# abowman6/CBET_RayTracing_3D

Hardware: AMD Instinct MI355X
Metric: ray-steps/sec, OMEGA 60-beam 256^3 sweep (higher is better)
Workload: dtype f64

## Files before the change

### cbet_raytracing_3d_amd/api.py

```python
import ctypes as C
import os

import numpy as np

_PKG = os.path.dirname(os.path.abspath(__file__))
LIB_PATH = os.environ.get("CBET_LIB_PATH") or os.path.join(_PKG, "lib", "libcbet_mi355x.so")
DATA_DIR = os.path.join(_PKG, "data")

OK, EINVAL, EHIP, ENOMEM, ENODEVICE, ECOMM = 0, -1, -2, -3, -4, -5
NPHASE = 2001
KERNEL_DEFAULT, KERNEL_GLOBAL_ATOMICS, KERNEL_LDS_COMBINE, KERNEL_LDS_WINDOW = 0, 1, 2, 3


class CbetError(RuntimeError):
    def __init__(self, code, msg):
        super().__init__("cbet error %d: %s" % (code, msg))
        self.code = code


class Params(C.Structure):
    _fields_ = [
        ("nx", C.c_int), ("ny", C.c_int), ("nz", C.c_int),
        ("xmin", C.c_double), ("xmax", C.c_double),
        ("ymin", C.c_double), ("ymax", C.c_double),
# ... 94 lines not shown

    def idx(c, n):
        c = np.where(c > 0.0, c, 0.0)
        return np.minimum(np.floor(c), n - 1).astype(np.int64)

    hist = np.zeros((ntheta, nphi))
    np.add.at(hist, (idx(ct, ntheta), idx(cp, nphi)), r["uray"])
    return hist


EXPORTS = [
    "cbet_last_error", "cbet_version", "cbet_params_default", "cbet_derive",
    "cbet_live_ray_list", "cbet_omega60_beam_norm", "cbet_host_power_table", "cbet_host_beam_trig", "cbet_read_profile",
    "cbet_safeGPUAlloc", "cbet_moveToAndFromGPU", "cbet_gpuFree",
    "cbet_context_create", "cbet_context_destroy", "cbet_context_counters", "cbet_context_tables", "cbet_context_set_launch_list",
    "cbet_launch_ray_XYZ", "cbet_tabulate_plasma", "cbet_trace_nodes", "cbet_prepare_step_records", "cbet_ray_tracing",
    "cbet_write_text", "cbet_edep_average", "cbet_edep_average_device", "cbet_node_coordinates", "cbet_write_npy",
    "cbet_debug_bounds_violations",
    "cbet_gain_params_default", "cbet_gain_constants", "cbet_trace_cbet", "cbet_gain_field",
    "cbet_cbet_workspace_bytes", "cbet_cbet_solve", "cbet_gain_field_slab", "cbet_gain_field_packed",
    "cbet_cbet_slab_workspace_bytes", "cbet_cbet_slab_workspace_bytes_parts", "cbet_pack_segments", "cbet_unpack_segments",
    "cbet_context_list_length", "cbet_cbet_workspace_gain", "cbet_trace_exits", "cbet_exit_tally", "cbet_farfield",
    "cbet_sph_modes_device", "cbet_sph_modes", "cbet_prepare_plasma", "cbet_context_step_records",
]

_lib = None


def lib():
    global _lib
    if _lib is not None:
        return _lib
    import torch
    if not os.path.exists(LIB_PATH):
        raise ImportError(
            "%s is missing: build it with `python -m cbet_raytracing_3d_amd.build` "
            "(hipcc --offload-arch=gfx950).  There is no CPU fallback." % LIB_PATH)
    L = C.CDLL(LIB_PATH)
    vp, dp, ip = C.c_void_p, C.POINTER(C.c_double), C.POINTER(C.c_int)
    L.cbet_last_error.restype = C.c_char_p
    L.cbet_version.restype = C.c_char_p
    L.cbet_params_default.argtypes = [C.POINTER(Params), C.c_int]
    L.cbet_derive.argtypes = [C.POINTER(Params), C.POINTER(Derived)]
    L.cbet_live_ray_list.argtypes = [C.POINTER(Params), ip, C.c_long, C.POINTER(C.c_long)]
    L.cbet_omega60_beam_norm.restype = dp
    L.cbet_host_power_table.argtypes = [dp, dp]
    L.cbet_host_beam_trig.argtypes = [dp, C.c_int, dp]
    L.cbet_read_profile.argtypes = [C.c_char_p, C.c_int, dp, dp]
    L.cbet_safeGPUAlloc.argtypes = [C.POINTER(vp), C.c_size_t, C.c_int]
    L.cbet_moveToAndFromGPU.argtypes = [vp, vp, C.c_size_t, C.c_int]
    L.cbet_gpuFree.argtypes = [vp, C.c_int]
    L.cbet_context_create.argtypes = [C.POINTER(vp), C.POINTER(Params), C.c_int]
    L.cbet_context_destroy.argtypes = [vp]
    L.cbet_context_counters.argtypes = [vp, vp, C.POINTER(Counters), C.c_int]
    L.cbet_context_set_launch_list.argtypes = [vp, ip, C.c_long]
    L.cbet_context_tables.argtypes = [vp, C.POINTER(vp), C.POINTER(vp)]
    L.cbet_launch_ray_XYZ.argtypes = [C.c_int, C.c_uint, vp, vp, vp, vp, vp, vp, vp, vp,
                                      C.c_double, C.c_double, C.c_double, C.POINTER(Params), vp, vp]
    L.cbet_tabulate_plasma.argtypes = [vp, C.POINTER(Params), vp, vp, vp, vp]
    L.cbet_prepare_step_records.argtypes = [vp, C.POINTER(Params), vp, vp, C.c_double, C.c_double, C.c_double, vp]
    L.cbet_prepare_plasma.argtypes = [vp, C.POINTER(Params), vp, vp, vp, C.c_double, C.c_double, C.c_double, vp]
    L.cbet_context_step_records.argtypes = [vp, C.POINTER(vp), C.POINTER(C.c_ulonglong)]
    L.cbet_trace_nodes.argtypes = [C.c_int, C.c_uint, vp, vp, vp, vp, vp, vp, vp,
                                   C.c_double, C.c_double, C.c_double, C.POINTER(Params), vp, vp]
    L.cbet_ray_tracing.argtypes = [dp, dp, dp, dp, C.POINTER(Params), dp, ip, C.c_int, dp,
                                   C.POINTER(Counters)]
    L.cbet_debug_bounds_violations.argtypes = [C.POINTER(C.c_ulonglong), C.c_int, vp]
    L.cbet_write_text.argtypes = [dp, C.c_int, C.c_int, C.c_int, C.c_char_p]
    L.cbet_write_text.restype = C.c_longlong
    L.cbet_edep_average.argtypes = [dp, dp, C.c_int, C.c_int, C.c_int]
    L.cbet_edep_average_device.argtypes = [vp, vp, C.c_int, C.c_int, C.c_int, vp]
    L.cbet_node_coordinates.argtypes = [C.POINTER(Params), dp, dp, dp]
    L.cbet_write_npy.argtypes = [dp, C.c_int, C.POINTER(C.c_long), C.c_char_p]
    L.cbet_write_npy.restype = C.c_longlong
    L.cbet_gain_params_default.argtypes = [C.POINTER(GainParams)]
    L.cbet_gain_constants.argtypes = [C.POINTER(Params), C.POINTER(GainParams), dp, dp, dp]
    L.cbet_trace_cbet.argtypes = [C.c_int, C.c_uint, vp, vp, vp, C.c_int, vp, vp, vp, vp, vp, vp,
                                  C.c_double, C.c_double, C.c_double, C.POINTER(Params), C.POINTER(GainParams), vp, vp]
    L.cbet_gain_field.argtypes = [vp, vp, vp, vp, vp, C.POINTER(Params), C.POINTER(GainParams), vp, vp]
    L.cbet_gain_field_slab.argtypes = [vp, vp, vp, vp, vp, C.c_int, C.c_int, C.POINTER(Params), C.POINTER(GainParams), vp, vp]
    L.cbet_gain_field_packed.argtypes = [vp, vp, vp, vp, vp, C.c_int, C.c_int, C.POINTER(Params), C.POINTER(GainParams), vp, vp]
    L.cbet_pack_segments.argtypes = [vp, C.c_long, C.c_int, C.c_int, vp, C.c_long, vp, vp]
    L.cbet_unpack_segments.argtypes = [vp, C.c_long, C.c_int, C.c_int, vp, C.c_long, vp, vp]
    L.cbet_cbet_slab_workspace_bytes.argtypes = [C.POINTER(Params), C.c_int, C.c_int]
    L.cbet_cbet_slab_workspace_bytes.restype = C.c_size_t
# ... 145 lines not shown
        c = Counters()
        _check(lib().cbet_context_counters(self._h, _addr(stream), C.byref(c), 1 if reset else 0))
        return c

    def set_launch_list(self, slots):
        arr = np.ascontiguousarray(slots, dtype=np.int32)
        _check(lib().cbet_context_set_launch_list(self._h, arr.ctypes.data_as(C.POINTER(C.c_int)), arr.size))

    def list_length(self):
        n = C.c_long()
        _check(lib().cbet_context_list_length(self._h, C.byref(n)))
        return n.value

    def tables(self):
        a, b = C.c_void_p(), C.c_void_p()
        _check(lib().cbet_context_tables(self._h, C.byref(a), C.byref(b)))
        return a.value, b.value

    def step_records(self):
        a, n = C.c_void_p(), C.c_ulonglong()
        _check(lib().cbet_context_step_records(self._h, C.byref(a), C.byref(n)))
        return a.value, n.value

    def close(self):
        if self._h:
            lib().cbet_context_destroy(self._h)
            self._h = C.c_void_p()

    def __del__(self):
        try:
            self.close()
        except Exception:
            pass


def launch_ray_XYZ(b, nindices, te_data_g, r_data_g, ne_data_g, edep, bbeam_norm, beam_norm, pow_r,
                   phase_r, xconst, yconst, zconst, params, ctx=None, stream=None):
    _check(lib().cbet_launch_ray_XYZ(
        b, nindices, _addr(te_data_g), _addr(r_data_g), _addr(ne_data_g), _addr(edep),
        _addr(bbeam_norm), _addr(beam_norm), _addr(pow_r), _addr(phase_r), xconst, yconst, zconst,
        C.byref(params), ctx.handle if ctx is not None else None, _addr(stream)))


def tabulate_plasma(ctx, params, te_data_g, r_data_g, ne_data_g, stream=None):
    _check(lib().cbet_tabulate_plasma(ctx.handle, C.byref(params), _addr(te_data_g),
                                      _addr(r_data_g), _addr(ne_data_g), _addr(stream)))
# ... 207 lines not shown
```

### cbet_raytracing_3d_amd/build.py

```python
import os
import shutil
import subprocess
import sys

PKG = os.path.dirname(os.path.abspath(__file__))
ROOT = os.path.dirname(PKG)
CSRC = os.path.join(PKG, "csrc")
LIB_DIR = os.path.join(PKG, "lib")
LIB_PATH = os.path.join(LIB_DIR, "libcbet_mi355x.so")
SOURCES = ["cbet_kernels.hip", "cbet_trace_window.hip", "cbet_trace_exit.hip", "cbet_grid_kernels.hip", "cbet_sph_modes.hip",
           "cbet_abi.cpp", "cbet_host.cpp", "cbet_output.cpp", "cbet_sph_host.cpp"]
HEADERS = [os.path.join(CSRC, "cbet_device.h"), os.path.join(CSRC, "cbet_relocate.h"), os.path.join(CSRC, "cbet_trace_common.h"), os.path.join(ROOT, "include", "cbet_mi355x.h"),
           os.path.join(ROOT, "include", "cbet_omega_beams.h")]

FLAGS = ["-O3", "-std=c++17", "--offload-arch=gfx950", "-ffp-contract=off", "-fPIC", "-shared",
         "-Wall", "-Wextra", "-Wno-unused-result", "-mllvm", "-structurizecfg-skip-uniform-regions=true"]


def hipcc():
    exe = shutil.which("hipcc") or "/opt/rocm/bin/hipcc"
    if not os.path.exists(exe):
        raise RuntimeError("hipcc not found (need ROCm to build the gfx950 library)")
    return exe


def is_stale():
    if not os.path.exists(LIB_PATH):
        return True
    built = os.path.getmtime(LIB_PATH)
    deps = [os.path.join(CSRC, s) for s in SOURCES] + HEADERS + [os.path.abspath(__file__),
                                                                os.path.join(ROOT, "tools", "cbet_gpu.cpp"),
                                                                os.path.join(ROOT, "tools", "cbet_reference_shaped.cpp"),
                                                                os.path.join(ROOT, "include", "cbet_reference_api.hpp")]
    return any(os.path.getmtime(d) > built for d in deps)

# ... 67 lines not shown
```

### cbet_raytracing_3d_amd/csrc/cbet_abi.cpp

```cpp
#include <hip/hip_runtime_api.h>

#include <algorithm>
#include <cmath>
#include <cstdarg>
#include <cstdio>
#include <cstdlib>
#include <cstring>
#include <map>
#include <mutex>
#include <vector>

#include "cbet_device.h"
#include "cbet_mi355x.h"
#include "cbet_omega_beams.h"

namespace cbet {

thread_local char g_err[512] = "";

int fail(int code, const char *fmt, ...)
{
    va_list ap;
    va_start(ap, fmt);
    vsnprintf(g_err, sizeof g_err, fmt, ap);
    va_end(ap);
    if (code == CBET_EHIP || code == CBET_ENODEVICE || code == CBET_ENOMEM) (void)hipGetLastError();
    return code;
}

#define CBET_HIP(call)                                                                          \
    do {                                                                                        \
        hipError_t e_ = (call);                                                                 \
        if (e_ != hipSuccess)                                                                   \
            return ::cbet::fail(CBET_EHIP, "%s failed: %s", #call, hipGetErrorString(e_));      \
    } while (0)
// ... 191 lines not shown
    xl = launch_axis(d->nrays_x, d->nrays_x, d->dx / 2);
    yl = launch_axis(d->nrays_y, d->nrays_y, d->dy / 2);
    long ntraced = 0, nlive = 0;
    build_live_list(p, d, d->nindices, xl, yl, live, ntraced, nlive);
    d->ntraced_ids = ntraced;
    d->nlive_rays = nlive;
    return CBET_OK;
}

}

using namespace cbet;

struct cbet_context {
    int gpu = -1;
    cbet_params p{};
    cbet_derived d{};
    double *ne3d = nullptr, *kap3d = nullptr;
    StepRecord *steprec = nullptr;
    unsigned long long tables_version = 0, rec_version = ~0ull;
    unsigned long long rec_builds = 0;
    const double *rec_ne3d = nullptr, *rec_kap3d = nullptr;
    double rec_const[3] = {0, 0, 0};
    double *xlaunch = nullptr, *ylaunch = nullptr;
    double *bounds = nullptr;
    int *live = nullptr;
    int nlive = 0;
    unsigned long long *counters = nullptr;
};

extern "C" {

const char *cbet_last_error(void) { return g_err; }
const char *cbet_version(void) { return "cbet-mi355x 0.1 (gfx950, hip)"; }

int cbet_params_default(cbet_params *p, int n)
{
    if (!p) return fail(CBET_EINVAL, "params is NULL");
    std::memset(p, 0, sizeof *p);
    p->nx = p->ny = p->nz = n;
    p->xmin = p->ymin = p->zmin = -0.13;
    p->xmax = p->ymax = p->zmax = 0.13;
    p->nbeams = 60;
    p->rays_per_zone = 4;
    p->courant_mult = 0.5;
    p->absorption = 1;
// ... 102 lines not shown
    if (e != hipSuccess) return fail(CBET_ENODEVICE, "hipSetDevice(%d): %s", gpu, hipGetErrorString(e));
    e = hipMemcpy(dst, src, size, hipMemcpyDefault);
    if (e != hipSuccess) return fail(CBET_EHIP, "Error encountered during hipMemcpy: %s", hipGetErrorString(e));
    return CBET_OK;
}

int cbet_gpuFree(void *ptr, int gpu)
{
    DeviceGuard guard;
    hipError_t e = hipSetDevice(gpu);
    if (e != hipSuccess) return fail(CBET_ENODEVICE, "hipSetDevice(%d): %s", gpu, hipGetErrorString(e));
    CBET_HIP(hipFree(ptr));
    return CBET_OK;
}

int cbet_context_destroy(cbet_context *ctx)
{
    if (!ctx) return CBET_OK;
    DeviceGuard guard;
    (void)hipSetDevice(ctx->gpu);
    (void)hipFree(ctx->ne3d);
    (void)hipFree(ctx->kap3d);
    (void)hipFree(ctx->steprec);
    (void)hipFree(ctx->xlaunch);
    (void)hipFree(ctx->ylaunch);
    (void)hipFree(ctx->bounds);
    (void)hipFree(ctx->live);
    (void)hipFree(ctx->counters);
    delete ctx;
    return CBET_OK;
}

int cbet_context_set_launch_list(cbet_context *ctx, const int *list, long n)
{
    if (!ctx || !list) return fail(CBET_EINVAL, "NULL context or list");
    if (n <= 0 || n % kWave != 0) return fail(CBET_EINVAL, "a launch list is a whole number of 64-entry bundles (got %ld entries)", n);
    DeviceGuard guard;
    CBET_HIP(hipSetDevice(ctx->gpu));
    CBET_HIP(hipDeviceSynchronize());
    std::vector<int> cur((size_t)ctx->nlive), want, got;
    if (ctx->nlive) CBET_HIP(hipMemcpy(cur.data(), ctx->live, cur.size() * sizeof(int), hipMemcpyDeviceToHost));
    for (int v : cur) if (v >= 0) want.push_back(v);
    for (long i = 0; i < n; ++i) {
        if (list[i] >= 0) got.push_back(list[i]);
        else if (list[i] != -1) return fail(CBET_EINVAL, "launch list entry %ld is %d (a ray id or -1)", i, list[i]);
    }
    for (long b = 0; b < n; b += kWave) {
        bool any = false;
        for (int l = 0; l < kWave; ++l) any = any || list[b + l] >= 0;
        if (!any) return fail(CBET_EINVAL, "bundle %ld of the launch list is empty", b / kWave);
    }
    std::sort(want.begin(), want.end());
    std::sort(got.begin(), got.end());
    if (want != got) return fail(CBET_EINVAL, "the launch list must hold exactly the context's live rays, each once (%zu given, %zu expected)", got.size(), want.size());
    int *fresh = nullptr;
    CBET_HIP(hipMalloc((void **)&fresh, (size_t)n * sizeof(int)));
    hipError_t e = hipMemcpy(fresh, list, (size_t)n * sizeof(int), hipMemcpyHostToDevice);
    if (e != hipSuccess) { (void)hipFree(fresh); return fail(CBET_EHIP, "hipMemcpy(launch list): %s", hipGetErrorString(e)); }
    (void)hipFree(ctx->live);
    ctx->live = fresh;
    ctx->nlive = (int)n;
    return CBET_OK;
}

int cbet_context_create(cbet_context **out, const cbet_params *p, int gpu)
{
    if (!out) return fail(CBET_EINVAL, "ctx out-pointer is NULL");
    *out = nullptr;
    if (int rc = validate(p)) return rc;
    cbet_derived d;
    std::vector<double> xl, yl;
    std::vector<int> live;
    if (int rc = derive_launch(p, &d, xl, yl, live)) return rc;

    DeviceGuard guard;
    hipError_t e = hipSetDevice(gpu);
    if (e != hipSuccess) return fail(CBET_ENODEVICE, "hipSetDevice(%d): %s", gpu, hipGetErrorString(e));
    cbet_context *ctx = new cbet_context;
    ctx->gpu = gpu;
    ctx->p = *p;
    ctx->d = d;
    ctx->nlive = (int)live.size();
    const size_t nodes = (size_t)p->nx * p->ny * p->nz;
    auto bail = [&](hipError_t err, const char *what) {
// ... 145 lines not shown
    if (int rc = check_geometry(ctx, p)) return rc;
    DeviceGuard guard;
    CBET_HIP(hipSetDevice(ctx->gpu));
    return step_records(ctx, p, ne3d, kappa3d, xconst, yconst, zconst, stream, true);
}

int cbet_prepare_plasma(cbet_context *ctx, const cbet_params *p, const double *te_data_g, const double *r_data_g,
                        const double *ne_data_g, double xconst, double yconst, double zconst, void *stream)
{
    if (!ctx) return fail(CBET_EINVAL, "NULL context");
    if (int rc = validate(p)) return rc;
    if (int rc = check_geometry(ctx, p)) return rc;
    if (!te_data_g || !r_data_g || !ne_data_g) return fail(CBET_EINVAL, "NULL profile pointer");
    if (plasma_records_lds(p->nprofile) > 65536) {
        if (int rc = cbet_tabulate_plasma(ctx, p, te_data_g, r_data_g, ne_data_g, stream)) return rc;
        return cbet_prepare_step_records(ctx, p, nullptr, nullptr, xconst, yconst, zconst, stream);
    }
    DeviceGuard guard;
    CBET_HIP(hipSetDevice(ctx->gpu));
    PlasmaRecordsArgs a{};
    a.t = tabulate_args(p, ctx, te_data_g, r_data_g, ne_data_g);
    a.xconst = xconst; a.yconst = yconst; a.zconst = zconst;
    a.rec = ctx->steprec;
    CBET_HIP(launch_plasma_records(a, (hipStream_t)stream));
    ++ctx->tables_version;
    ++ctx->rec_builds;
    ctx->rec_version = ctx->tables_version;
    ctx->rec_ne3d = ctx->ne3d; ctx->rec_kap3d = ctx->kap3d;
    ctx->rec_const[0] = xconst; ctx->rec_const[1] = yconst; ctx->rec_const[2] = zconst;
    return CBET_OK;
}

struct CbetHooks {
    const double *gain = nullptr;
    int quantity = 0;
    double *beam_gain = nullptr;
    double max_exponent = 0.0;
    bool exits = false;
};

static int trace_impl(int b, unsigned nindices, const double *ne3d, const double *kappa3d,
                      double *edep, const double *bbeam_norm, const double *beam_norm,
                      const double *pow_r, const double *phase_r, double xconst, double yconst,
                      double zconst, const cbet_params *p, cbet_context *ctx, void *stream,
                      const CbetHooks &hooks)
{
// ... 455 lines not shown
```

### cbet_raytracing_3d_amd/csrc/cbet_device.h

```cpp
#ifndef CBET_DEVICE_H_
#define CBET_DEVICE_H_

#include <hip/hip_runtime_api.h>

#include "cbet_mi355x.h"

namespace cbet {

constexpr double kC = 29979245800.0;
constexpr double kE0 = 8.85418782e-12;
constexpr double kMe = 9.10938356e-31;
constexpr double kEc = 1.60217662e-19;
constexpr double kLambda = 1.053e-4 / 3.0;
constexpr double kSigma = 0.0375;
constexpr double kIntensity = 1.0e14;
constexpr double kFocal = 0.1;
constexpr double kBeamMin = -450.0e-4;
constexpr double kBeamMax = 450.0e-4;

constexpr unsigned kEmptyTag = 0xFFFFFFFFu;
constexpr int kWave = 64;

enum CounterSlot { kCntSteps = 0, kCntRays = 1, kCntGlobalAtomics = 2, kCntEvictions = 3, kCntWaveSteps = 4,
                   kCntWaveStepsMiss = 5, kCntWaveStepsWide = 6, kCntSlabsRetired = 7, kCntSlots = 8 };
// ... 2 lines not shown
    int nx, ny, nz, nprofile;
    double xmin, ymin, zmin;
    double dx, dy, dz, dt;
    double ncrit;
    const double *r, *ne, *te;
    double *ne3d, *kap3d;
};

struct StepRecord {
    double kx, ky, kz, kap;
};

struct StepTableArgs {
    int nx, ny, nz;
    double xconst, yconst, zconst;
    const double *ne3d, *kap3d;
    StepRecord *rec;
};

struct PlasmaRecordsArgs {
    TabulateArgs t;
    double xconst, yconst, zconst;
    StepRecord *rec;
};

struct TraceArgs {
    int nx, ny, nz;
    double xmin, ymin, zmin;
    double dx, dy, dz, dt;
    double inv_dx, inv_dy, inv_dz;
    double fx_hi, fy_hi, fz_hi;
    const double *bounds;
    double tol_x, tol_y, tol_z;
    double xconst, yconst, zconst;
    int nt, absorption;
    int rpz, zones, nrays_x;
    double z_launch;
    double uray_mult, omega, ncrit;
    const double *xlaunch, *ylaunch;
    const int *live;
    int nlive;
    int beam_lo, nbeams_local, bundles_per_beam;
    long total_bundles;
    long first_item, item_count;
    const double *ne3d, *kap3d;
    const StepRecord *steprec;
// ... 73 lines not shown
```

### cbet_raytracing_3d_amd/csrc/cbet_kernels.hip

```cpp
#include <hip/hip_runtime.h>

#include "cbet_trace_common.h"

namespace cbet {
namespace {

__device__ __forceinline__ void interp_table2(const double *y1, const double *y2, const double *x, const double xp,
                                              int n, double &o1, double &o2)
{
    const bool ascending = x[0] <= x[n - 1];
    if (ascending ? (xp <= x[0]) : (xp >= x[0])) { o1 = y1[0]; o2 = y2[0]; return; }
    if (ascending ? (xp >= x[n - 1]) : (xp <= x[n - 1])) { o1 = y1[n - 1]; o2 = y2[n - 1]; return; }
    unsigned lo = 0, hi = n - 1, mid = (lo + hi) >> 1;
    while (lo < hi - 1) {
        const bool go_low = ascending ? (x[mid] >= xp) : !(x[mid] <= xp);
        if (go_low) hi = mid; else lo = mid;
        mid = (lo + hi) >> 1;
    }
    const double dx = x[mid + 1] - x[mid], t = xp - x[mid];
    o1 = y1[mid] + (y1[mid + 1] - y1[mid]) / dx * t;
    o2 = y2[mid] + (y2[mid + 1] - y2[mid]) / dx * t;
}

__device__ __forceinline__ void node_plasma(const TabulateArgs &a, const double *s_r, const double *s_ne, const double *s_te,
// ... 39 lines not shown
    const long sY = a.nz, sX = (long)a.ny * a.nz;
    for (long idx = (long)blockIdx.x * blockDim.x + threadIdx.x; idx < total; idx += stride) {
        const int k = (int)(idx % a.nz);
        const long ij = idx / a.nz;
        const int j = (int)(ij % a.ny);
        const int i = (int)(ij / a.ny);
        const long oxm = (i == 0) ? 0 : ((i == a.nx - 1) ? -2 * sX : -sX), oxp = (i == 0) ? 2 * sX : ((i == a.nx - 1) ? 0 : sX);
        const long oym = (j == 0) ? 0 : ((j == a.ny - 1) ? -2 * sY : -sY), oyp = (j == 0) ? 2 * sY : ((j == a.ny - 1) ? 0 : sY);
        const long ozm = (k == 0) ? 0 : ((k == a.nz - 1) ? -2 : -1), ozp = (k == 0) ? 2 : ((k == a.nz - 1) ? 0 : 1);
        StepRecord r;
        r.kx = a.xconst * (a.ne3d[idx + oxp] - a.ne3d[idx + oxm]);
        r.ky = a.yconst * (a.ne3d[idx + oyp] - a.ne3d[idx + oym]);
        r.kz = a.zconst * (a.ne3d[idx + ozp] - a.ne3d[idx + ozm]);
        r.kap = a.kap3d[idx];
        a.rec[idx] = r;
    }
}

constexpr int kPrTY = 8, kPrTZ = 64, kPrXC = 16, kPrThreads = 256;
constexpr int kPrPZ = kPrTZ + 2;
constexpr int kPrPlane = (kPrTY + 2) * kPrPZ;
constexpr int kPrTile = kPrTY * kPrTZ;
constexpr int kPrItems = kPrTile + 2 * kPrTZ + 2 * kPrTY;

__global__ void __launch_bounds__(kPrThreads) k_plasma_records(const PlasmaRecordsArgs a)
{
    extern __shared__ double s_prof[];
    const TabulateArgs &t = a.t;
    double *s_r = s_prof, *s_ne = s_prof + t.nprofile, *s_te = s_prof + 2 * t.nprofile;
    double *s_ring = s_prof + 3 * t.nprofile;
    double *s_kap = s_ring + 3 * kPrPlane;
    const int tid = threadIdx.x;
    for (int i = tid; i < t.nprofile; i += kPrThreads) {
        s_r[i] = t.r[i];
        s_ne[i] = t.ne[i];
        s_te[i] = t.te[i];
    }
    __syncthreads();
    const int nx = t.nx, ny = t.ny, nz = t.nz;
    const int k0 = max(0, min((int)blockIdx.x * kPrTZ, nz - kPrTZ));
    const int j0 = max(0, min((int)blockIdx.y * kPrTY, ny - kPrTY));
    const int x0 = (int)blockIdx.z * kPrXC, x1 = min(x0 + kPrXC, nx);
    const int pa = x0 == 0 ? 0 : min(x0 - 1, nx - 3);
    const int pb = x1 == nx ? nx : max(x1 + 1, 3);

    auto emit = [&](int i, int xl, int xh) {
        const double *lo = s_ring + (xl % 3) * kPrPlane, *hi = s_ring + (xh % 3) * kPrPlane, *mid = s_ring + (i % 3) * kPrPlane;
        const double *kap = s_kap + (i % 3) * kPrTile;
        for (int q = tid; q < 2 * kPrTile; q += kPrThreads) {
            const int n = q >> 1, jr = n / kPrTZ, kr = n % kPrTZ;
            const int j = j0 + jr, k = k0 + kr;
            if (j >= ny || k >= nz) continue;
            const int c = (jr + 1) * kPrPZ + kr + 1;
            double v0, v1;
            if ((q & 1) == 0) {
                const int ym = (j == 0) ? 0 : ((j == ny - 1) ? -2 : -1), yp = (j == 0) ? 2 : ((j == ny - 1) ? 0 : 1);
                v0 = a.xconst * (hi[c] - lo[c]);
                v1 = a.yconst * (mid[c + yp * kPrPZ] - mid[c + ym * kPrPZ]);
            } else {
                const int zm = (k == 0) ? 0 : ((k == nz - 1) ? -2 : -1), zp = (k == 0) ? 2 : ((k == nz - 1) ? 0 : 1);
                v0 = a.zconst * (mid[c + zp] - mid[c + zm]);
                v1 = kap[n];
            }
            const long idx = ((long)i * ny + j) * nz + k;
            reinterpret_cast<double2 *>(a.rec + idx)[q & 1] = make_double2(v0, v1);
        }
    };

    for (int p = pa; p < pb; ++p) {
        const bool own_plane = p >= x0 && p < x1;
        double *ring = s_ring + (p % 3) * kPrPlane;
        for (int n = tid; n < (own_plane ? kPrItems : kPrTile); n += kPrThreads) {
            int jj, kk;
            if (n < kPrTile) {
                jj = 1 + n / kPrTZ; kk = 1 + n % kPrTZ;
            } else if (n < kPrTile + 2 * kPrTZ) {
                const int h = n - kPrTile;
                jj = h < kPrTZ ? 0 : kPrTY + 1; kk = 1 + h % kPrTZ;
            } else {
                const int h = n - kPrTile - 2 * kPrTZ;
                kk = h < kPrTY ? 0 : kPrTZ + 1; jj = 1 + h % kPrTY;
            }
            const int j = j0 + jj - 1, k = k0 + kk - 1;
            if (j < 0 || j >= ny || k < 0 || k >= nz) continue;
            double ed, kap;
            if (own_plane && n < kPrTile) {
                node_plasma(t, s_r, s_ne, s_te, p, j, k, ed, kap);
                s_kap[(p % 3) * kPrTile + n] = kap;
                const long idx = ((long)p * ny + j) * nz + k;
                t.ne3d[idx] = ed;
                t.kap3d[idx] = kap;
            } else {
                node_plasma(t, s_r, s_ne, s_te, p, j, k, ed, kap);
            }
            ring[jj * kPrPZ + kk] = ed;
        }
        __syncthreads();
        if (p == 2 && x0 == 0) emit(0, 0, 2);
        if (p - 1 >= 1 && p - 1 >= x0 && p - 1 < x1) emit(p - 1, p - 2, p);
        if (p == nx - 1 && x1 == nx) emit(nx - 1, nx - 3, nx - 1);
        __syncthreads();
    }
}

template <int WL>
struct LdsWindow {
    static constexpr int W = 1 << WL;
    static constexpr int NSLOT = W * W * W;
    double *val;
    unsigned *tag;
    const TraceArgs *args;

    __device__ __forceinline__ unsigned slot(int i, int j, int k) const
    {
        return (unsigned)((((i & (W - 1)) << WL) | (j & (W - 1))) << WL | (k & (W - 1)));
    }
    __device__ __forceinline__ void clear(int lane)
    {
        for (int s = lane; s < NSLOT; s += kWave) {
            val[s] = 0.0;
            tag[s] = kEmptyTag;
        }
    }
    __device__ __forceinline__ void add(unsigned s, double w)
// ... 187 lines not shown
}

hipError_t launch_tabulate(const TabulateArgs &a, hipStream_t stream)
{
    const long total = (long)a.nx * a.ny * a.nz;
    long blocks = (total + 255) / 256;
    if (blocks > 256 * 16) blocks = 256 * 16;
    const size_t lds = sizeof(double) * 3 * (size_t)a.nprofile;
    hipLaunchKernelGGL(k_tabulate, dim3((unsigned)blocks), dim3(256), lds, stream, a);
    return hipGetLastError();
}

hipError_t launch_step_table(const StepTableArgs &a, hipStream_t stream)
{
    const long total = (long)a.nx * a.ny * a.nz;
    long blocks = (total + 255) / 256;
    if (blocks > 256 * 16) blocks = 256 * 16;
    hipLaunchKernelGGL(k_step_table, dim3((unsigned)blocks), dim3(256), 0, stream, a);
    return hipGetLastError();
}

size_t plasma_records_lds(int nprofile)
{
    return sizeof(double) * (3 * (size_t)nprofile + 3 * (size_t)kPrPlane + 3 * (size_t)kPrTile);
}

hipError_t launch_plasma_records(const PlasmaRecordsArgs &a, hipStream_t stream)
{
    const dim3 grid((unsigned)((a.t.nz + kPrTZ - 1) / kPrTZ), (unsigned)((a.t.ny + kPrTY - 1) / kPrTY),
                    (unsigned)((a.t.nx + kPrXC - 1) / kPrXC));
    hipLaunchKernelGGL(k_plasma_records, grid, dim3(kPrThreads), plasma_records_lds(a.t.nprofile), stream, a);
    return hipGetLastError();
}

hipError_t audit_violations(unsigned long long *out, bool reset, hipStream_t stream)
{
#ifdef CBET_DEBUG_BOUNDS
    hipError_t e = hipStreamSynchronize(stream);
    if (e != hipSuccess) return e;
    e = hipMemcpyFromSymbol(out, HIP_SYMBOL(g_audit_violations), sizeof *out);
    if (e == hipSuccess && reset) {
        const unsigned long long zero = 0;
        e = hipMemcpyToSymbol(HIP_SYMBOL(g_audit_violations), &zero, sizeof zero);
    }
    return e;
#else
    (void)out; (void)reset; (void)stream;
// ... 31 lines not shown
```

### cbet_raytracing_3d_amd/pipeline.py

```python
import os

import torch

from . import api


def row_pitch(nz, pad_rows):
    if int(pad_rows) > nz + 2:
        return int(pad_rows)
    return -(-(nz + 2) // 8) * 8 if pad_rows else nz + 2


def all_reduce_staged(t, group=None):
    import torch.distributed as dist
    if t.is_cuda and dist.get_backend(group) != "nccl":
        t = t.cpu()
    dist.all_reduce(t, op=dist.ReduceOp.SUM, group=group)
    return t


def allreduce_grid(edep, group=None, force=False):
    import torch.distributed as dist
    if dist.is_available() and dist.is_initialized() and (dist.get_world_size(group) > 1 or force):
        total = all_reduce_staged(edep, group)
# ... 2 lines not shown
    return edep


def reduce_scatter_grid(grid, slab, group=None, async_op=False, force=False):
    import torch.distributed as dist
    if not (dist.is_available() and dist.is_initialized()) or (dist.get_world_size(group) == 1 and not force):
        slab.copy_(grid[: slab.shape[0]])
        return None
    if dist.get_backend(group) == "nccl":
        return dist.reduce_scatter_tensor(slab, grid, op=dist.ReduceOp.SUM, group=group, async_op=async_op)
    total = all_reduce_staged(grid, group)
    r, pl = dist.get_rank(group), slab.shape[0]
    slab.copy_(total[r * pl:(r + 1) * pl])
    return None


class SweepPipeline:

    def __init__(self, tracer, rank=0, world_size=1, group=None, overlap_traces=None, force_collectives=False, pad_rows=None):
        self.tr, self.rank, self.world, self.group = tracer, rank, world_size, group
        self.force = force_collectives
        self.overlap_traces = True if overlap_traces is None else bool(overlap_traces)
        p = tracer.params
        self.ctx = [tracer.ctx, api.Context(p, tracer.gpu)]
        planes = -(-(p.nx + 2) // world_size) * world_size
        if pad_rows is None:
            pad_rows = int(os.environ.get("CBET_PAD_ROWS", "1"))
        zp = row_pitch(p.nz, pad_rows)
        shape = (planes, p.ny + 2, zp)
        dev = tracer.device
        self.grids = [torch.zeros(shape, dtype=torch.float64, device=dev) for _ in range(2)]
        self.slab_store = [torch.zeros((planes // world_size,) + shape[1:], dtype=torch.float64, device=dev) for _ in range(2)]
        self.slabs = [s[..., : p.nz + 2] for s in self.slab_store]
        self.s_prep = [torch.cuda.Stream(device=dev) for _ in range(2)]
        self.s_trace = [torch.cuda.Stream(device=dev) for _ in range(2)]
        if not self.overlap_traces:
            self.s_trace[1] = self.s_trace[0]
        self.ev_prep = [torch.cuda.Event() for _ in range(2)]
        self.ev_consumed = [None, None]
        self.ev_trace = [None, None]
        self.work = [None, None]
        self.kernel_events = []
        from .tracer import shard_of_rank
        si, sc = shard_of_rank(rank, world_size)
        self.launch_p = p.copy(beam_lo=0, beam_hi=p.nbeams, shard_index=si, shard_count=sc,
                               edep_zpitch=zp if pad_rows else 0)
        self.passes = 0

    def run_pass(self, timed=False):
        tr, b = self.tr, self.passes % 2
        self.passes += 1
        with torch.cuda.stream(self.s_prep[b]):
            if self.ev_trace[b] is not None:
                self.s_prep[b].wait_event(self.ev_trace[b])
            if self.work[b] is not None:
                self.work[b].wait()
                self.work[b] = None
            self.grids[b].zero_()
            tr._prepare_plasma(self.launch_p, self.ctx[b])
            self.ev_prep[b].record()
        with torch.cuda.stream(self.s_trace[b]):
            self.s_trace[b].wait_event(self.ev_prep[b])
            if timed:
                e0, e1 = torch.cuda.Event(enable_timing=True), torch.cuda.Event(enable_timing=True)
                e0.record()
            tr._trace(self.grids[b], self.launch_p, self.ctx[b])
            if timed:
                e1.record()
                self.kernel_events.append((e0, e1))
            consumed, self.ev_consumed[b] = self.ev_consumed[b], None
            if consumed is not None:
                self.s_trace[b].wait_event(consumed)
            self.work[b] = reduce_scatter_grid(self.grids[b], self.slab_store[b], self.group, async_op=True, force=self.force)
            self.ev_trace[b] = torch.cuda.Event()
            self.ev_trace[b].record()
        return b

    def wait_combined(self, b):
        cur = torch.cuda.current_stream(self.tr.device)
        if self.work[b] is not None:
            self.work[b].wait()
        if self.ev_trace[b] is not None:
            cur.wait_event(self.ev_trace[b])

    def release(self, b):
        ev = torch.cuda.Event()
        ev.record(torch.cuda.current_stream(self.tr.device))
        self.ev_consumed[b] = ev

    def time_trace_alone(self, reps=3):
        tr = self.tr
        self.finish()
        times = []
        with torch.cuda.stream(self.s_trace[0]):
            for _ in range(reps + 1):
                self.grids[0].zero_()
# ... 46 lines not shown
```

### cbet_raytracing_3d_amd/tracer.py

```python
import numpy as np
import torch

from . import api
from .cbet_loop import (_DeviceCbetEngine, _agree, _frozen, _parts, balanced_slabs, cbet_fixed_point,
                        cbet_fixed_point_slabs, gain_update_weights, slab_pieces)
from .exchange import SegmentPlan, _pack_rows_cpu, _segment_rows, _SlabExchanger
from .pipeline import SweepPipeline, allreduce_grid, reduce_scatter_grid, row_pitch


def _require(t, shape, what):
    if t.dtype != torch.float64 or not t.is_contiguous() or tuple(t.shape) != tuple(shape):
        raise ValueError("%s must be a contiguous float64 tensor of shape %s" % (what, tuple(shape)))


class RayTracer:

    def __init__(self, params, r_profile, ne_profile, te_profile, beam_norm=None, device=None):
        if not torch.cuda.is_available():
            raise RuntimeError("RayTracer needs a HIP device (no CPU fallback)")
        self.device = torch.device("cuda", torch.cuda.current_device()) if device is None \
            else torch.device(device)
        self.gpu = self.device.index if self.device.index is not None else torch.cuda.current_device()
        self.params = params.copy()
        self.derived = api.derive(self.params)
        if beam_norm is None:
            beam_norm = api.omega60_beam_norm()[: self.params.nbeams]
        beam_norm = np.ascontiguousarray(beam_norm, dtype=np.float64).reshape(-1, 3)
        if beam_norm.shape[0] != self.params.nbeams:
            raise ValueError("beam_norm has %d rows, params.nbeams=%d" % (beam_norm.shape[0], self.params.nbeams))
        phase_r, pow_r = api.host_power_table()
        bbeam = api.host_beam_trig(beam_norm)

        def up(a):
            return torch.from_numpy(np.ascontiguousarray(a, dtype=np.float64)).to(self.device)

        self.d_beam_norm, self.d_bbeam_norm = up(beam_norm), up(bbeam)
        self.d_pow_r, self.d_phase_r = up(pow_r), up(phase_r)
        self.d_r, self.d_ne, self.d_te = up(r_profile), up(ne_profile), up(te_profile)
        for t in (self.d_r, self.d_ne, self.d_te):
            if t.numel() != self.params.nprofile:
                raise ValueError("profile length != params.nprofile")
        self.ctx = api.Context(self.params, self.gpu)
        self._launch_list = None
        self.grid_shape = (self.params.nx + 2, self.params.ny + 2, self.params.nz + 2)

    def _stream(self):
        return torch.cuda.current_stream(self.device).cuda_stream

    def _grad_consts(self):
        d = self.derived
        return d.xconst, d.yconst, d.zconst

    def _tail(self, host_trig=True):
        return (self.d_bbeam_norm if host_trig else None, self.d_beam_norm, self.d_pow_r, self.d_phase_r) + self._grad_consts()

    def _trace(self, out, params, ctx=None):
        api.trace_nodes(0, self.derived.nindices, None, None, out, *self._tail(), params, self.ctx if ctx is None else ctx,
                        self._stream())

    def _prepare_plasma(self, params, ctx):
        api.prepare_plasma(ctx, params, self.d_te, self.d_r, self.d_ne, *self._grad_consts(), self._stream())

    def _prepare_step_records(self):
        api.prepare_step_records(self.ctx, self.params, None, None, *self._grad_consts(), self._stream())

    def new_grid(self, per_beam=False, zpitch=None):
        if zpitch:
# ... 185 lines not shown
```

### include/cbet_mi355x.h

```cpp
#ifndef CBET_MI355X_H_
#define CBET_MI355X_H_

#include <stddef.h>

#ifdef __cplusplus
extern "C" {
#endif

#define CBET_OK 0
#define CBET_EINVAL (-1)
#define CBET_EHIP (-2)
#define CBET_ENOMEM (-3)
#define CBET_ENODEVICE (-4)
#define CBET_ECOMM (-5)

#define CBET_NPHASE 2001
#define CBET_MAX_CBET_BEAMS 64

#define CBET_KERNEL_DEFAULT 0
#define CBET_KERNEL_GLOBAL_ATOMICS 1
#define CBET_KERNEL_LDS_COMBINE 2
#define CBET_KERNEL_LDS_WINDOW 3

#define CBET_BEAMS_BY_GPU (-1)
// ... 56 lines not shown
const char *cbet_version(void);

int cbet_params_default(cbet_params *p, int n);
int cbet_derive(const cbet_params *p, cbet_derived *d);

int cbet_live_ray_list(const cbet_params *p, int *out, long cap, long *count);

const double *cbet_omega60_beam_norm(void);
int cbet_host_power_table(double *phase_r, double *pow_r);
int cbet_host_beam_trig(const double *beam_norm, int nbeams, double *bbeam_norm);
int cbet_read_profile(const char *path, int nprofile, double *r, double *v);

int cbet_safeGPUAlloc(void **dst, size_t size, int gpu);
int cbet_moveToAndFromGPU(void *dst, void *src, size_t size, int gpu);
int cbet_gpuFree(void *ptr, int gpu);

int cbet_context_create(cbet_context **ctx, const cbet_params *p, int gpu);
int cbet_context_destroy(cbet_context *ctx);
int cbet_context_counters(cbet_context *ctx, void *stream, cbet_counters *out, int reset);
int cbet_context_set_launch_list(cbet_context *ctx, const int *list, long n);
int cbet_context_list_length(const cbet_context *ctx, long *length);
int cbet_context_tables(cbet_context *ctx, double **ne3d, double **kappa3d);
int cbet_context_step_records(const cbet_context *ctx, const void **records, unsigned long long *builds);

int cbet_debug_bounds_violations(unsigned long long *out, int reset, void *stream);

int cbet_launch_ray_XYZ(int b, unsigned nindices, double *te_data_g, double *r_data_g,
                        double *ne_data_g, double *edep, double *bbeam_norm, double *beam_norm,
                        double *pow_r, double *phase_r, double xconst, double yconst,
                        double zconst, const cbet_params *p, cbet_context *ctx, void *stream);

int cbet_tabulate_plasma(cbet_context *ctx, const cbet_params *p, const double *te_data_g,
                         const double *r_data_g, const double *ne_data_g, void *stream);
int cbet_trace_nodes(int b, unsigned nindices, const double *ne3d, const double *kappa3d,
                     double *edep, const double *bbeam_norm, const double *beam_norm,
                     const double *pow_r, const double *phase_r, double xconst, double yconst,
                     double zconst, const cbet_params *p, cbet_context *ctx, void *stream);
int cbet_prepare_step_records(cbet_context *ctx, const cbet_params *p, const double *ne3d,
                              const double *kappa3d, double xconst, double yconst, double zconst,
                              void *stream);
int cbet_prepare_plasma(cbet_context *ctx, const cbet_params *p, const double *te_data_g,
                        const double *r_data_g, const double *ne_data_g, double xconst, double yconst,
                        double zconst, void *stream);

int cbet_ray_tracing(const double *te_profile, const double *r_profile, const double *ne_profile,
                     double *edep, const cbet_params *p, const double *beam_norm, const int *gpus,
// ... 116 lines not shown
```

Before: 168.1 billion.

## Use bucketed direct interval lookup and precomputed slopes in plasma records kernel

Replaces the per-node binary search over the radial profile with a bucket table (built on the host at context setup) followed by a short bounded walk. It also precomputes interpolation slopes in LDS, keeps kappa in registers rather than a three-plane LDS ring, and in single-GPU runs skips the reduce-scatter by aliasing the slab store to the grids. The aim is to cut search, divide and LDS cost during plasma preparation and to drop a redundant collective. The cost is extra host-side setup and an assumption that the device profile still matches the abscissae given at setup, which is only checked in debug builds.

```diff
diff --git a/cbet_raytracing_3d_amd/api.py b/cbet_raytracing_3d_amd/api.py
--- a/cbet_raytracing_3d_amd/api.py
+++ b/cbet_raytracing_3d_amd/api.py
@@ -140,6 +140,7 @@
     "cbet_cbet_slab_workspace_bytes", "cbet_cbet_slab_workspace_bytes_parts", "cbet_pack_segments", "cbet_unpack_segments",
     "cbet_context_list_length", "cbet_cbet_workspace_gain", "cbet_trace_exits", "cbet_exit_tally", "cbet_farfield",
     "cbet_sph_modes_device", "cbet_sph_modes", "cbet_prepare_plasma", "cbet_context_step_records",
+    "cbet_context_set_profile",
 ]
 
 _lib = None
@@ -179,6 +180,7 @@
     L.cbet_prepare_step_records.argtypes = [vp, C.POINTER(Params), vp, vp, C.c_double, C.c_double, C.c_double, vp]
     L.cbet_prepare_plasma.argtypes = [vp, C.POINTER(Params), vp, vp, vp, C.c_double, C.c_double, C.c_double, vp]
     L.cbet_context_step_records.argtypes = [vp, C.POINTER(vp), C.POINTER(C.c_ulonglong)]
+    L.cbet_context_set_profile.argtypes = [vp, vp, dp, C.c_int, ip, ip]
     L.cbet_trace_nodes.argtypes = [C.c_int, C.c_uint, vp, vp, vp, vp, vp, vp, vp,
                                    C.c_double, C.c_double, C.c_double, C.POINTER(Params), vp, vp]
     L.cbet_ray_tracing.argtypes = [dp, dp, dp, dp, C.POINTER(Params), dp, ip, C.c_int, dp,
@@ -370,6 +372,16 @@
         _check(lib().cbet_context_step_records(self._h, C.byref(a), C.byref(n)))
         return a.value, n.value
 
+    def set_profile(self, r_data_g, r_host):
+        direct, walk = C.c_int(0), C.c_int(0)
+        if r_host is None:
+            _check(lib().cbet_context_set_profile(self._h, None, None, 0, None, None))
+            return False, 0
+        arr = np.ascontiguousarray(r_host, dtype=np.float64)
+        _check(lib().cbet_context_set_profile(self._h, _addr(r_data_g), arr.ctypes.data_as(C.POINTER(C.c_double)), arr.size,
+                                              C.byref(direct), C.byref(walk)))
+        return bool(direct.value), walk.value
+
     def close(self):
         if self._h:
             lib().cbet_context_destroy(self._h)
diff --git a/cbet_raytracing_3d_amd/build.py b/cbet_raytracing_3d_amd/build.py
--- a/cbet_raytracing_3d_amd/build.py
+++ b/cbet_raytracing_3d_amd/build.py
@@ -10,7 +10,7 @@
 LIB_PATH = os.path.join(LIB_DIR, "libcbet_mi355x.so")
 SOURCES = ["cbet_kernels.hip", "cbet_trace_window.hip", "cbet_trace_exit.hip", "cbet_grid_kernels.hip", "cbet_sph_modes.hip",
            "cbet_abi.cpp", "cbet_host.cpp", "cbet_output.cpp", "cbet_sph_host.cpp"]
-HEADERS = [os.path.join(CSRC, "cbet_device.h"), os.path.join(CSRC, "cbet_relocate.h"), os.path.join(CSRC, "cbet_trace_common.h"), os.path.join(ROOT, "include", "cbet_mi355x.h"),
+HEADERS = [os.path.join(CSRC, "cbet_device.h"), os.path.join(CSRC, "cbet_relocate.h"), os.path.join(CSRC, "cbet_interval_search.h"), os.path.join(CSRC, "cbet_trace_common.h"), os.path.join(ROOT, "include", "cbet_mi355x.h"),
            os.path.join(ROOT, "include", "cbet_omega_beams.h")]
 
 FLAGS = ["-O3", "-std=c++17", "--offload-arch=gfx950", "-ffp-contract=off", "-fPIC", "-shared",
diff --git a/cbet_raytracing_3d_amd/csrc/cbet_abi.cpp b/cbet_raytracing_3d_amd/csrc/cbet_abi.cpp
--- a/cbet_raytracing_3d_amd/csrc/cbet_abi.cpp
+++ b/cbet_raytracing_3d_amd/csrc/cbet_abi.cpp
@@ -11,6 +11,7 @@
 #include <vector>
 
 #include "cbet_device.h"
+#include "cbet_interval_search.h"
 #include "cbet_mi355x.h"
 #include "cbet_omega_beams.h"
 
@@ -248,6 +249,10 @@
     unsigned long long rec_builds = 0;
     const double *rec_ne3d = nullptr, *rec_kap3d = nullptr;
     double rec_const[3] = {0, 0, 0};
+    const double *search_r = nullptr;
+    int search_n = 0;
+    double search_inv_w = 0.0;
+    unsigned short *search_first = nullptr;
     double *xlaunch = nullptr, *ylaunch = nullptr;
     double *bounds = nullptr;
     int *live = nullptr;
@@ -396,6 +401,7 @@
     (void)hipFree(ctx->ne3d);
     (void)hipFree(ctx->kap3d);
     (void)hipFree(ctx->steprec);
+    (void)hipFree(ctx->search_first);
     (void)hipFree(ctx->xlaunch);
     (void)hipFree(ctx->ylaunch);
     (void)hipFree(ctx->bounds);
@@ -434,6 +440,35 @@
     (void)hipFree(ctx->live);
     ctx->live = fresh;
     ctx->nlive = (int)n;
+    return CBET_OK;
+}
+
+int cbet_context_set_profile(cbet_context *ctx, const double *r_data_g, const double *r_host, int nprofile, int *direct,
+                             int *max_walk)
+{
+    if (!ctx) return fail(CBET_EINVAL, "NULL context");
+    if (direct) *direct = 0;
+    if (max_walk) *max_walk = 0;
+    if (r_host && !r_data_g) return fail(CBET_EINVAL, "NULL device profile pointer");
+    if (r_host && nprofile != ctx->p.nprofile)
+        return fail(CBET_EINVAL, "the context was created for %d profile rows, not %d", ctx->p.nprofile, nprofile);
+    ctx->search_r = nullptr;
+    if (!r_host) return CBET_OK;
+    std::vector<unsigned short> first(kSearchBuckets);
+    double inv_w;
+    int walk;
+    const bool admitted = interval_plan(r_host, nprofile, first.data(), &inv_w, &walk);
+    if (max_walk) *max_walk = walk;
+    if (!admitted) return CBET_OK;
+    DeviceGuard guard;
+    CBET_HIP(hipSetDevice(ctx->gpu));
+    CBET_HIP(hipDeviceSynchronize());
+    if (!ctx->search_first) CBET_HIP(hipMalloc((void **)&ctx->search_first, kSearchBuckets * sizeof(unsigned short)));
+    CBET_HIP(hipMemcpy(ctx->search_first, first.data(), kSearchBuckets * sizeof(unsigned short), hipMemcpyHostToDevice));
+    ctx->search_r = r_data_g;
+    ctx->search_n = nprofile;
+    ctx->search_inv_w = inv_w;
+    if (direct) *direct = 1;
     return CBET_OK;
 }
 
@@ -625,6 +660,25 @@
     a.t = tabulate_args(p, ctx, te_data_g, r_data_g, ne_data_g);
     a.xconst = xconst; a.yconst = yconst; a.zconst = zconst;
     a.rec = ctx->steprec;
+    if (ctx->search_r && ctx->search_r == r_data_g && ctx->search_n == p->nprofile) {
+#ifdef CBET_DEBUG_BOUNDS
+        {
+            std::vector<double> r((size_t)p->nprofile);
+            std::vector<unsigned short> first(kSearchBuckets), declared(kSearchBuckets);
+            CBET_HIP(hipMemcpyAsync(r.data(), r_data_g, r.size() * sizeof(double), hipMemcpyDeviceToHost, (hipStream_t)stream));
+            CBET_HIP(hipMemcpyAsync(declared.data(), ctx->search_first, declared.size() * sizeof(unsigned short), hipMemcpyDeviceToHost,
+                                    (hipStream_t)stream));
+            CBET_HIP(hipStreamSynchronize((hipStream_t)stream));
+            double inv_w;
+            int walk;
+            if (!interval_plan(r.data(), p->nprofile, first.data(), &inv_w, &walk) || inv_w != ctx->search_inv_w || first != declared)
+                return fail(CBET_EINVAL, "r_data_g no longer holds the abscissae cbet_context_set_profile was given");
+        }
+#endif
+        a.direct = 1;
+        a.inv_w = ctx->search_inv_w;
+        a.first = ctx->search_first;
+    }
     CBET_HIP(launch_plasma_records(a, (hipStream_t)stream));
     ++ctx->tables_version;
     ++ctx->rec_builds;
diff --git a/cbet_raytracing_3d_amd/csrc/cbet_device.h b/cbet_raytracing_3d_amd/csrc/cbet_device.h
--- a/cbet_raytracing_3d_amd/csrc/cbet_device.h
+++ b/cbet_raytracing_3d_amd/csrc/cbet_device.h
@@ -48,6 +48,9 @@
     TabulateArgs t;
     double xconst, yconst, zconst;
     StepRecord *rec;
+    int direct;
+    double inv_w;
+    const unsigned short *first;
 };
 
 struct TraceArgs {
diff --git a/cbet_raytracing_3d_amd/csrc/cbet_interval_search.h b/cbet_raytracing_3d_amd/csrc/cbet_interval_search.h
--- /dev/null
+++ b/cbet_raytracing_3d_amd/csrc/cbet_interval_search.h
@@ -0,0 +1,66 @@
+#ifndef CBET_INTERVAL_SEARCH_H_
+#define CBET_INTERVAL_SEARCH_H_
+
+#include <math.h>
+
+#if defined(__HIPCC__)
+#define CBET_IS_HD __host__ __device__ __forceinline__
+#else
+#define CBET_IS_HD static inline
+#endif
+
+namespace cbet {
+
+constexpr int kSearchBuckets = 1024;
+constexpr int kSearchMaxWalk = 16;
+
+CBET_IS_HD int interval_bisect(const double *x, int n, bool ascending, double xp)
+{
+    unsigned lo = 0, hi = n - 1, mid = (lo + hi) >> 1;
+    while (lo < hi - 1) {
+        const bool go_low = ascending ? (x[mid] >= xp) : !(x[mid] <= xp);
+        if (go_low) hi = mid; else lo = mid;
+        mid = (lo + hi) >> 1;
+    }
+    return (int)mid;
+}
+
+CBET_IS_HD int interval_bucket(double x0, double inv_w, double xp)
+{
+    const double f = (xp - x0) * inv_w;
+    return f < (double)(kSearchBuckets - 1) ? (int)f : kSearchBuckets - 1;
+}
+
+CBET_IS_HD int interval_direct(const double *x, int n, const unsigned short *first, double inv_w, double xp)
+{
+    int m = first[interval_bucket(x[0], inv_w, xp)];
+    while (m > 0 && x[m] >= xp) --m;
+    while (m < n - 2 && !(x[m + 1] >= xp)) ++m;
+    return m;
+}
+
+static inline bool interval_plan(const double *x, int n, unsigned short *first, double *inv_w, int *max_walk)
+{
+    *inv_w = 0.0;
+    *max_walk = 0;
+    if (n < 2 || n > 65536) return false;
+    for (int i = 0; i + 1 < n; ++i)
+        if (!(x[i] < x[i + 1])) return false;
+    const double inv = (double)kSearchBuckets / (x[n - 1] - x[0]);
+    if (!isfinite(x[0]) || !isfinite(x[n - 1]) || !isfinite(inv) || !(inv > 0.0)) return false;
+    int b = 0;
+    for (int m = 0; m <= n - 2; ++m)
+        for (const int top = (m == n - 2) ? kSearchBuckets - 1 : interval_bucket(x[0], inv, x[m + 1]); b <= top; ++b)
+            first[b] = (unsigned short)m;
+    int longest = 0;
+    b = kSearchBuckets - 1;
+    for (int m = n - 2; m >= 0; --m)
+        for (const int bottom = (m == 0) ? 0 : interval_bucket(x[0], inv, x[m]); b >= bottom; --b)
+            if (m - (int)first[b] > longest) longest = m - (int)first[b];
+    *inv_w = inv;
+    *max_walk = longest;
+    return longest <= kSearchMaxWalk;
+}
+
+}
+#endif
diff --git a/cbet_raytracing_3d_amd/csrc/cbet_kernels.hip b/cbet_raytracing_3d_amd/csrc/cbet_kernels.hip
--- a/cbet_raytracing_3d_amd/csrc/cbet_kernels.hip
+++ b/cbet_raytracing_3d_amd/csrc/cbet_kernels.hip
@@ -1,5 +1,6 @@
 #include <hip/hip_runtime.h>
 
+#include "cbet_interval_search.h"
 #include "cbet_trace_common.h"
 
 namespace cbet {
@@ -85,21 +86,63 @@
 constexpr int kPrPlane = (kPrTY + 2) * kPrPZ;
 constexpr int kPrTile = kPrTY * kPrTZ;
 constexpr int kPrItems = kPrTile + 2 * kPrTZ + 2 * kPrTY;
+constexpr int kPrOwn = kPrTile / kPrThreads;
+static_assert(kPrTile % kPrThreads == 0, "a thread keeps kappa of kPrOwn tile nodes per plane");
+
+struct StagedProfile {
+    const double *r, *ne, *te, *s_ne, *s_te;
+    const unsigned short *first;
+};
+
+__device__ __forceinline__ void node_plasma_staged(const PlasmaRecordsArgs &a, const StagedProfile &s, int i, int j, int k,
+                                                   double &ed, double &kap)
+{
+    const TabulateArgs &t = a.t;
+    const int n = t.nprofile;
+    const double xc = i * t.dx + t.xmin, yc = j * t.dy + t.ymin, zc = k * t.dz + t.zmin;
+    const double rho = sqrt(xc * xc + yc * yc + zc * zc);
+    const bool ascending = s.r[0] <= s.r[n - 1];
+    double etemp;
+    if (ascending ? (rho <= s.r[0]) : (rho >= s.r[0])) {
+        ed = s.ne[0]; etemp = s.te[0];
+    } else if (ascending ? (rho >= s.r[n - 1]) : (rho <= s.r[n - 1])) {
+        ed = s.ne[n - 1]; etemp = s.te[n - 1];
+    } else {
+        const int mid = a.direct ? interval_direct(s.r, n, s.first, a.inv_w, rho) : interval_bisect(s.r, n, ascending, rho);
+        const double tt = rho - s.r[mid];
+        ed = s.ne[mid] + s.s_ne[mid] * tt;
+        etemp = s.te[mid] + s.s_te[mid] * tt;
+    }
+    const double eta = 5.2e-5 * 10.0 / (etemp * sqrt(etemp));
+    const double nuei = (1e6 * ed * (kEc * kEc) / kMe) * eta;
+    kap = ed / t.ncrit * nuei * t.dt;
+}
 
 __global__ void __launch_bounds__(kPrThreads) k_plasma_records(const PlasmaRecordsArgs a)
 {
     extern __shared__ double s_prof[];
     const TabulateArgs &t = a.t;
-    double *s_r = s_prof, *s_ne = s_prof + t.nprofile, *s_te = s_prof + 2 * t.nprofile;
-    double *s_ring = s_prof + 3 * t.nprofile;
+    const int np = t.nprofile;
+    double *s_r = s_prof, *s_ne = s_prof + np, *s_te = s_prof + 2 * np, *s_sne = s_prof + 3 * np, *s_ste = s_prof + 4 * np;
+    double *s_ring = s_prof + 5 * np;
     double *s_kap = s_ring + 3 * kPrPlane;
+    unsigned short *s_first = reinterpret_cast<unsigned short *>(s_kap + kPrTile);
     const int tid = threadIdx.x;
-    for (int i = tid; i < t.nprofile; i += kPrThreads) {
+    for (int i = tid; i < np; i += kPrThreads) {
         s_r[i] = t.r[i];
         s_ne[i] = t.ne[i];
         s_te[i] = t.te[i];
     }
+    if (a.direct)
+        for (int i = tid; i < kSearchBuckets; i += kPrThreads) s_first[i] = a.first[i];
     __syncthreads();
+    for (int i = tid; i < np - 1; i += kPrThreads) {
+        const double dx = s_r[i + 1] - s_r[i];
+        s_sne[i] = (s_ne[i + 1] - s_ne[i]) / dx;
+        s_ste[i] = (s_te[i + 1] - s_te[i]) / dx;
+    }
+    __syncthreads();
+    const StagedProfile prof{s_r, s_ne, s_te, s_sne, s_ste, s_first};
     const int nx = t.nx, ny = t.ny, nz = t.nz;
     const int k0 = max(0, min((int)blockIdx.x * kPrTZ, nz - kPrTZ));
     const int j0 = max(0, min((int)blockIdx.y * kPrTY, ny - kPrTY));
@@ -107,9 +150,14 @@
     const int pa = x0 == 0 ? 0 : min(x0 - 1, nx - 3);
     const int pb = x1 == nx ? nx : max(x1 + 1, 3);
 
+    double kap_p[kPrOwn] = {}, kap_p1[kPrOwn] = {}, kap_p2[kPrOwn] = {};
+    auto stage_kappa = [&](const double (&kp)[kPrOwn]) {
+#pragma unroll
+        for (int it = 0; it < kPrOwn; ++it) s_kap[tid + it * kPrThreads] = kp[it];
+    };
+
     auto emit = [&](int i, int xl, int xh) {
         const double *lo = s_ring + (xl % 3) * kPrPlane, *hi = s_ring + (xh % 3) * kPrPlane, *mid = s_ring + (i % 3) * kPrPlane;
-        const double *kap = s_kap + (i % 3) * kPrTile;
         for (int q = tid; q < 2 * kPrTile; q += kPrThreads) {
             const int n = q >> 1, jr = n / kPrTZ, kr = n % kPrTZ;
             const int j = j0 + jr, k = k0 + kr;
@@ -123,19 +171,29 @@
             } else {
                 const int zm = (k == 0) ? 0 : ((k == nz - 1) ? -2 : -1), zp = (k == 0) ? 2 : ((k == nz - 1) ? 0 : 1);
                 v0 = a.zconst * (mid[c + zp] - mid[c + zm]);
-                v1 = kap[n];
+                v1 = s_kap[n];
             }
             const long idx = ((long)i * ny + j) * nz + k;
             reinterpret_cast<double2 *>(a.rec + idx)[q & 1] = make_double2(v0, v1);
         }
+    };
+    auto emit_face = [&](int i, int xl, int xh, const double (&kp)[kPrOwn]) {
+        __syncthreads();
+        stage_kappa(kp);
+        __syncthreads();
+        emit(i, xl, xh);
     };
 
     for (int p = pa; p < pb; ++p) {
         const bool own_plane = p >= x0 && p < x1;
         double *ring = s_ring + (p % 3) * kPrPlane;
-        for (int n = tid; n < (own_plane ? kPrItems : kPrTile); n += kPrThreads) {
+        stage_kappa(kap_p1);
+#pragma unroll
+        for (int it = 0; it < (kPrItems + kPrThreads - 1) / kPrThreads; ++it) {
+            const int n = tid + it * kPrThreads;
+            if (n >= (own_plane ? kPrItems : kPrTile)) continue;
             int jj, kk;
-            if (n < kPrTile) {
+            if (it < kPrOwn) {
                 jj = 1 + n / kPrTZ; kk = 1 + n % kPrTZ;
             } else if (n < kPrTile + 2 * kPrTZ) {
                 const int h = n - kPrTile;
@@ -147,22 +205,27 @@
             const int j = j0 + jj - 1, k = k0 + kk - 1;
             if (j < 0 || j >= ny || k < 0 || k >= nz) continue;
             double ed, kap;
-            if (own_plane && n < kPrTile) {
-                node_plasma(t, s_r, s_ne, s_te, p, j, k, ed, kap);
-                s_kap[(p % 3) * kPrTile + n] = kap;
+            if (own_plane && it < kPrOwn) {
+                node_plasma_staged(a, prof, p, j, k, ed, kap);
+                kap_p[it] = kap;
                 const long idx = ((long)p * ny + j) * nz + k;
                 t.ne3d[idx] = ed;
                 t.kap3d[idx] = kap;
             } else {
-                node_plasma(t, s_r, s_ne, s_te, p, j, k, ed, kap);
+                node_plasma_staged(a, prof, p, j, k, ed, kap);
             }
             ring[jj * kPrPZ + kk] = ed;
         }
         __syncthreads();
-        if (p == 2 && x0 == 0) emit(0, 0, 2);
         if (p - 1 >= 1 && p - 1 >= x0 && p - 1 < x1) emit(p - 1, p - 2, p);
-        if (p == nx - 1 && x1 == nx) emit(nx - 1, nx - 3, nx - 1);
+        if (p == 2 && x0 == 0) emit_face(0, 0, 2, kap_p2);
+        if (p == nx - 1 && x1 == nx) emit_face(nx - 1, nx - 3, nx - 1, kap_p);
         __syncthreads();
+#pragma unroll
+        for (int it = 0; it < kPrOwn; ++it) {
+            kap_p2[it] = kap_p1[it];
+            kap_p1[it] = kap_p[it];
+        }
     }
 }
 
@@ -396,7 +459,7 @@
 
 size_t plasma_records_lds(int nprofile)
 {
-    return sizeof(double) * (3 * (size_t)nprofile + 3 * (size_t)kPrPlane + 3 * (size_t)kPrTile);
+    return sizeof(double) * (5 * (size_t)nprofile + 3 * (size_t)kPrPlane + (size_t)kPrTile) + sizeof(unsigned short) * kSearchBuckets;
 }
 
 hipError_t launch_plasma_records(const PlasmaRecordsArgs &a, hipStream_t stream)
diff --git a/cbet_raytracing_3d_amd/pipeline.py b/cbet_raytracing_3d_amd/pipeline.py
--- a/cbet_raytracing_3d_amd/pipeline.py
+++ b/cbet_raytracing_3d_amd/pipeline.py
@@ -48,7 +48,7 @@
         self.force = force_collectives
         self.overlap_traces = True if overlap_traces is None else bool(overlap_traces)
         p = tracer.params
-        self.ctx = [tracer.ctx, api.Context(p, tracer.gpu)]
+        self.ctx = [tracer.ctx, tracer.new_context()]
         planes = -(-(p.nx + 2) // world_size) * world_size
         if pad_rows is None:
             pad_rows = int(os.environ.get("CBET_PAD_ROWS", "1"))
@@ -56,7 +56,9 @@
         shape = (planes, p.ny + 2, zp)
         dev = tracer.device
         self.grids = [torch.zeros(shape, dtype=torch.float64, device=dev) for _ in range(2)]
-        self.slab_store = [torch.zeros((planes // world_size,) + shape[1:], dtype=torch.float64, device=dev) for _ in range(2)]
+        self.local = world_size == 1 and not force_collectives
+        self.slab_store = self.grids if self.local else \
+            [torch.zeros((planes // world_size,) + shape[1:], dtype=torch.float64, device=dev) for _ in range(2)]
         self.slabs = [s[..., : p.nz + 2] for s in self.slab_store]
         self.s_prep = [torch.cuda.Stream(device=dev) for _ in range(2)]
         self.s_trace = [torch.cuda.Stream(device=dev) for _ in range(2)]
@@ -82,6 +84,10 @@
             if self.work[b] is not None:
                 self.work[b].wait()
                 self.work[b] = None
+            if self.local:
+                consumed, self.ev_consumed[b] = self.ev_consumed[b], None
+                if consumed is not None:
+                    self.s_prep[b].wait_event(consumed)
             self.grids[b].zero_()
             tr._prepare_plasma(self.launch_p, self.ctx[b])
             self.ev_prep[b].record()
@@ -94,10 +100,11 @@
             if timed:
                 e1.record()
                 self.kernel_events.append((e0, e1))
-            consumed, self.ev_consumed[b] = self.ev_consumed[b], None
-            if consumed is not None:
-                self.s_trace[b].wait_event(consumed)
-            self.work[b] = reduce_scatter_grid(self.grids[b], self.slab_store[b], self.group, async_op=True, force=self.force)
+            if not self.local:
+                consumed, self.ev_consumed[b] = self.ev_consumed[b], None
+                if consumed is not None:
+                    self.s_trace[b].wait_event(consumed)
+                self.work[b] = reduce_scatter_grid(self.grids[b], self.slab_store[b], self.group, async_op=True, force=self.force)
             self.ev_trace[b] = torch.cuda.Event()
             self.ev_trace[b].record()
         return b
diff --git a/cbet_raytracing_3d_amd/tracer.py b/cbet_raytracing_3d_amd/tracer.py
--- a/cbet_raytracing_3d_amd/tracer.py
+++ b/cbet_raytracing_3d_amd/tracer.py
@@ -40,9 +40,15 @@
         for t in (self.d_r, self.d_ne, self.d_te):
             if t.numel() != self.params.nprofile:
                 raise ValueError("profile length != params.nprofile")
-        self.ctx = api.Context(self.params, self.gpu)
+        self.r_profile = np.ascontiguousarray(r_profile, dtype=np.float64)
+        self.ctx = self.new_context()
         self._launch_list = None
         self.grid_shape = (self.params.nx + 2, self.params.ny + 2, self.params.nz + 2)
+
+    def new_context(self):
+        ctx = api.Context(self.params, self.gpu)
+        ctx.set_profile(self.d_r, self.r_profile)
+        return ctx
 
     def _stream(self):
         return torch.cuda.current_stream(self.device).cuda_stream
diff --git a/include/cbet_mi355x.h b/include/cbet_mi355x.h
--- a/include/cbet_mi355x.h
+++ b/include/cbet_mi355x.h
@@ -102,6 +102,8 @@
 int cbet_context_list_length(const cbet_context *ctx, long *length);
 int cbet_context_tables(cbet_context *ctx, double **ne3d, double **kappa3d);
 int cbet_context_step_records(const cbet_context *ctx, const void **records, unsigned long long *builds);
+int cbet_context_set_profile(cbet_context *ctx, const double *r_data_g, const double *r_host, int nprofile, int *direct,
+                             int *max_walk);
 
 int cbet_debug_bounds_violations(unsigned long long *out, int reset, void *stream);
 
```

After: 170.1 billion, median of 6. No clear change (+1.2%).
